# tomcreutz/slam-uwv_kalman_filters

Hardware: AMD Instinct MI355X
Metric: UKF predict+update steps/sec at batch=65536 PoseUKF instances, 1 & 8 GPU (higher is better)
Workload: dtype f64

## Files before the change

### slam-uwv_kalman_filters_amd/csrc/uwvk_psp_dev.hpp

```cpp
#pragma once
#include <cstddef>

#include "uwvk_pose_dev.hpp"
#include "uwvk_tiles.hpp"


#ifndef PSP_PAIR
#define PSP_PAIR 0
#endif
#ifndef PSP_NS
#define PSP_NS psp
#endif

namespace uwvk {
namespace PSP_NS {

constexpr int kLanes = PSP_PAIR ? 32 : 64;

UWVK_DEV void chain_prio_hi() { __builtin_amdgcn_s_setprio(1); }
UWVK_DEV void chain_prio_lo() { __builtin_amdgcn_s_setprio(0); }

template <int DOF>
struct PG {
  static constexpr int NP = DOF * (DOF + 1) / 2;
  static constexpr int NSLOT = (NP + kLanes - 1) / kLanes;
  static constexpr int N = 2 * DOF + 1;
  static constexpr int KP = 15;
  static constexpr int STG = 115;
};

template <int DOF>
struct alignas(16) PspSmem {
  double S[PG<DOF>::NP];
  double mu[Lay<DOF>::store];
  double stg[PG<DOF>::STG];
};
static_assert(sizeof(PspSmem<53>) <= 12800, "12 instances per CU");
static_assert(offsetof(PspSmem<53>, mu) == sizeof(double) * PG<53>::NP, "mu follows S");
static_assert(offsetof(PspSmem<53>, stg) == sizeof(double) * (PG<53>::NP + Lay<53>::store), "stg follows mu");
static_assert(offsetof(PspSmem<26>, mu) == sizeof(double) * PG<26>::NP, "mu follows S");
static_assert(offsetof(PspSmem<26>, stg) == sizeof(double) * (PG<26>::NP + Lay<26>::store), "stg follows mu");
constexpr int kPdLane0 = 27, kPdN = 27;
template <int DOF>
struct alignas(16) PspSmemPD : PspSmem<DOF> {
  double pS[32];
  double pm[32];
};
template <int DOF, int PD>
struct SmemT {
  using type = PspSmem<DOF>;
};
template <int DOF>
struct SmemT<DOF, 1> {
  using type = PspSmemPD<DOF>;
};
template <int DOF>
UWVK_DEV double* pd_ptr(PspSmem<DOF>&) {
  return nullptr;
}
template <int DOF>
UWVK_DEV double* pd_ptr(PspSmemPD<DOF>& s) {
  return s.pS;
}
UWVK_DEV constexpr int pd_dof(int d) { return d < 19 ? d : d + 27; }
UWVK_DEV constexpr int pd_store(int s) { return s < 20 ? s : s + 27; }

template <int DOF>
UWVK_DEV double* flat(PspSmem<DOF>& sm) {
  return reinterpret_cast<double*>(&sm);
}
template <int DOF>
UWVK_DEV const double* flat(const PspSmem<DOF>& sm) {
  return reinterpret_cast<const double*>(&sm);
}
template <int DOF>
constexpr int kFlatMu = PG<DOF>::NP;


UWVK_DEV int olane() {
  int l = PSP_PAIR ? ((int)threadIdx.x & 31) : (int)threadIdx.x;
  asm volatile("" : "+v"(l));
  return l;
}

template <class F>
UWVK_DEV constexpr unsigned long long lane_mask(F f) {
  unsigned long long m = 0;
  for (int i = 0; i < 64; i++)
    if (f(PSP_PAIR ? (i & 31) : i)) m |= 1ull << i;
  return m;
}
UWVK_DEV constexpr unsigned long long rep_mask(unsigned long long m) {
  return PSP_PAIR ? ((m & 0xFFFFFFFFull) | ((m & 0xFFFFFFFFull) << 32)) : m;
}
UWVK_DEV constexpr bool mask_needs_split(unsigned long long m) {
  return m >= 0xFFFFFFFF80000000ull && m < 0xFFFFFFFFFFFFFFF0ull;
}
UWVK_DEV bool lane_in_split(unsigned long long m) {
  unsigned lo = (unsigned)m, hi = (unsigned)(m >> 32);
  asm volatile("" : "+s"(lo), "+s"(hi));
  return __builtin_amdgcn_inverse_ballot_w64(((unsigned long long)hi << 32) | lo);
}
template <unsigned long long M>
UWVK_DEV bool lane_const() {
  if constexpr (mask_needs_split(M)) return lane_in_split(M);
  else return __builtin_amdgcn_inverse_ballot_w64(M);
}
#define LANE_IF(l, expr)                                                                                        \
  ({                                                                                                            \
    constexpr unsigned long long m_ = ::uwvk::PSP_NS::lane_mask([](int l) constexpr { return (bool)(expr); }); \
    ::uwvk::PSP_NS::lane_const<m_>();                                                                           \
  })
#define LANE_IN(m)                                                                     \
  (::uwvk::PSP_NS::mask_needs_split(::uwvk::PSP_NS::rep_mask(m))                       \
       ? ::uwvk::PSP_NS::lane_in_split(::uwvk::PSP_NS::rep_mask(m))                    \
       : __builtin_amdgcn_inverse_ballot_w64(::uwvk::PSP_NS::rep_mask(m)))
UWVK_DEV bool upper_half() { return lane_const<0xFFFFFFFF00000000ull>(); }
#if PSP_PAIR
template <int J>
UWVK_DEV double hbc(double v) {
  static_assert(J >= 0 && J < 16, "row_newbcast lane");
  int lo = __builtin_amdgcn_mov_dpp(__double2loint(v), 0x150 + J, 0xf, 0xf, false);
  int hi = __builtin_amdgcn_mov_dpp(__double2hiint(v), 0x150 + J, 0xf, 0xf, false);
  lo = __builtin_amdgcn_update_dpp(lo, lo, 0x142, 0xa, 0xf, false);
  hi = __builtin_amdgcn_update_dpp(hi, hi, 0x142, 0xa, 0xf, false);
  return __hiloint2double(hi, lo);
}
#endif
UWVK_DEV double hread(double v, int j) {
#if PSP_PAIR
  if (__builtin_constant_p(j) && j >= 0 && j < 16) {
    switch (j) {
      case 0: return hbc<0>(v);
      case 1: return hbc<1>(v);
      case 2: return hbc<2>(v);
      case 3: return hbc<3>(v);
      case 4: return hbc<4>(v);
      case 5: return hbc<5>(v);
      case 6: return hbc<6>(v);
      case 7: return hbc<7>(v);
      case 8: return hbc<8>(v);
      case 9: return hbc<9>(v);
      case 10: return hbc<10>(v);
      case 11: return hbc<11>(v);
      case 12: return hbc<12>(v);
      case 13: return hbc<13>(v);
      case 14: return hbc<14>(v);
      default: return hbc<15>(v);
    }
  }
  const double a = readlane_d(v, j), b = readlane_d(v, 32 + j);
  return upper_half() ? b : a;
#else
  return readlane_d(v, j);
#endif
}
UWVK_DEV int hlane(int j) { return PSP_PAIR ? j + ((int)threadIdx.x & 32) : j; }
UWVK_DEV constexpr int couple_c(int d) { return d < 3 ? d + 6 : (d >= 6 && d < 9 ? d + 3 : -1); }
template <int DOF>
UWVK_DEV constexpr unsigned long long col_ge_mask(int p, bool coupled) {
  unsigned long long m = 0;
  for (int l = 0; l < 64; l++) {
    const int jl = l < DOF ? l : DOF - 1, jc = couple_c(jl);
    const int j = coupled ? (jc >= 0 ? jc : jl) : jl;
    if (j >= p) m |= 1ull << l;
  }
  return m;
}
template <int DOF>
UWVK_DEV constexpr unsigned long long rows_store_mask(int p) {
  unsigned long long m = 0;
  for (int l = 0; l < 64; l++) {
    const int jl = l < DOF ? l : DOF - 1;
    if (!(couple_c(jl) >= 0) || l <= p) m |= 1ull << l;
  }
  return m;
}
template <class RL>
UWVK_DEV constexpr unsigned long long rows_mask() {
  unsigned long long m = 0;
  for (int k = 0; k < RL::NR; k++) m |= 1ull << RL::rows[k];
  return m;
}
template <class HM>
UWVK_DEV constexpr unsigned long long cols_mask() {
  unsigned long long m = 0;
  for (int k = 0; k < HM::NC; k++) m |= 1ull << HM::cols[k];
  for (int k = 1; k < HM::NC; k++)
    if (HM::cols[k] <= HM::cols[k - 1]) return 0;
  return m;
}
template <class RL>
UWVK_DEV constexpr bool rows_ascending() {
  for (int k = 1; k < RL::NR; k++)
    if (RL::rows[k] <= RL::rows[k - 1]) return false;
  return true;
}

template <int CTRL, int ROW, int BANK>
UWVK_DEV double dpp_d(double v) {
  const int lo = __builtin_amdgcn_update_dpp(0, __double2loint(v), CTRL, ROW, BANK, true);
  const int hi = __builtin_amdgcn_update_dpp(0, __double2hiint(v), CTRL, ROW, BANK, true);
  return __hiloint2double(hi, lo);
}
template <int NL = 64>
UWVK_DEV double wave_sum_dpp(double v) {
  double s = v + dpp_d<0x111, 0xf, 0xf>(v);
  s = s + dpp_d<0x112, 0xf, 0xf>(v);
  s = s + dpp_d<0x113, 0xf, 0xf>(v);
  s = s + dpp_d<0x114, 0xf, 0xe>(s);
  s = s + dpp_d<0x118, 0xf, 0xc>(s);
#if PSP_PAIR
  static_assert(NL <= 32, "pair: one instance per 32-lane half");
  if constexpr (NL <= 16) return hread(s, 15);
  s = s + dpp_d<0x142, 0xa, 0xf>(s);
  return hread(s, 31);
#else
  if constexpr (NL <= 16) return readlane_d(s, 15);
  s = s + dpp_d<0x142, 0xa, 0xf>(s);
  if constexpr (NL <= 32) return readlane_d(s, 31);
  s = s + dpp_d<0x143, 0xc, 0xf>(s);
  return readlane_d(s, 63);
#endif
}
UWVK_DEV double sk(double c) {
  asm volatile("" : "+s"(c));
  return c;
}
UWVK_DEV void so3_exp_psp(const double v[3], double o[4]) {
  const double t2 = v[0] * v[0] + v[1] * v[1] + v[2] * v[2];
  if (t2 < 0.0625) {
    const double u = 0.25 * t2;
    double s = u * sk(-1.0 / 39916800.0);
    s = s + sk(1.0 / 362880.0);
    s = fma(s, u, sk(-1.0 / 5040.0));
    s = fma(s, u, sk(1.0 / 120.0));
    s = fma(s, u, sk(-1.0 / 6.0));
    s = fma(s, u, 1.0);
    s = 0.5 * s;
    double c = u * sk(-1.0 / 3628800.0);
    c = c + sk(1.0 / 40320.0);
    c = fma(c, u, sk(-1.0 / 720.0));
    c = fma(c, u, sk(1.0 / 24.0));
    c = fma(c, u, -0.5);
    c = fma(c, u, 1.0);
    o[0] = c; o[1] = s * v[0]; o[2] = s * v[1]; o[3] = s * v[2];
  } else {
    so3_exp(v, o);
  }
}
UWVK_DEV void so3_log_psp(const double q[4], double o[3]) {
  double w = q[0], x = q[1], y = q[2], z = q[3];
  if (w < 0) { w = -w; x = -x; y = -y; z = -z; }
  const double n2 = x * x + y * y + z * z, w2 = w * w;
  if (n2 < 0.0025 * w2) {
    double iw = __builtin_amdgcn_rcp(w);
    iw = fma(iw, fma(-w, iw, 1.0), iw);
    iw = fma(iw, fma(-w, iw, 1.0), iw);
    const double r2 = n2 * (iw * iw);
    double a = r2 * sk(-1.0 / 13.0);
    a = fma(a, -r2, sk(1.0 / 11.0));
    a = fma(a, -r2, sk(1.0 / 9.0));
    a = fma(a, -r2, sk(1.0 / 7.0));
    a = fma(a, -r2, sk(1.0 / 5.0));
    a = fma(a, -r2, sk(1.0 / 3.0));
    a = fma(a, -r2, 1.0);
    const double k = 2.0 * a * iw;
    o[0] = k * x; o[1] = k * y; o[2] = k * z;
  } else {
    so3_log(q, o);
  }
}
template <int SR>
UWVK_DEV void qplus_psp(const double e[4], const double q[4], double o[4]) {
  if constexpr (SR) qmul(q, e, o);
  else qmul(e, q, o);
}
template <int SR>
UWVK_DEV void qboxminus_psp(const double a[4], const double b[4], double o[3]) {
  double bc[4] = {b[0], -b[1], -b[2], -b[3]}, r[4];
  if constexpr (SR) qmul(bc, a, r);
  else qmul(a, bc, r);
  so3_log_psp(r, o);
}

UWVK_DEV double swap_pair_d(double v) { return dpp_d<0xb1, 0xf, 0xf>(v); }

UWVK_DEV double sel3(double v0, double v1, double v2, int i) { return i == 0 ? v0 : (i == 1 ? v1 : v2); }
UWVK_DEV double sel6(double v0, double v1, double v2, double v3, double v4, double v5, int i) {
  return i < 3 ? sel3(v0, v1, v2, i) : sel3(v3, v4, v5, i - 3);
}

UWVK_DEV int pidx_sel(int p, int j, int Tj) { return j >= p ? Tj + p : p * (p + 1) / 2 + j; }
UWVK_DEV int pidx_sel_b(int p, int j, int Tj, bool ge) { return ge ? Tj + p : p * (p + 1) / 2 + j; }

UWVK_DEV void wsync() {
  __builtin_amdgcn_fence(__ATOMIC_RELEASE, "wavefront");
  __builtin_amdgcn_wave_barrier();
  __builtin_amdgcn_fence(__ATOMIC_ACQUIRE, "wavefront");
}

template <int R, int NL, int STRIDE>
UWVK_DEV void lds_sums(const double (&v)[R], double* buf, int l, double (&out)[R]) {
  static_assert(NL % 2 == 0 && R * NL <= 115, "transpose buffer (PG::STG)");
  const int c = l / STRIDE;
  if (l % STRIDE == 0 && c < NL) {
#pragma unroll
    for (int i = 0; i < R; i++) buf[i * NL + c] = v[i];
  }
  wsync();
  const double* row = buf + (l < R ? l : 0) * NL;
  double p[NL / 2];
#pragma unroll
  for (int k = 0; k < NL / 2; k++) p[k] = row[2 * k] + row[2 * k + 1];
#pragma unroll
  for (int w = 1; w < NL / 2; w *= 2)
#pragma unroll
    for (int k = 0; k + w < NL / 2; k += 2 * w) p[k] += p[k + w];
#pragma unroll
  for (int i = 0; i < R; i++) out[i] = hread(p[0], i);
}

#define PSP_PHASE(ph) \
  do {                \
    UWVK_STAMP(ph);   \
    l = olane();      \
  } while (0)

UWVK_DEV void psync() {
  __builtin_amdgcn_fence(__ATOMIC_RELEASE, "workgroup");
  __builtin_amdgcn_s_barrier();
  __builtin_amdgcn_fence(__ATOMIC_ACQUIRE, "workgroup");
}

UWVK_DEV constexpr bool scaled_dof(int d) { return d >= 12 && d != 18; }

template <int K, int J>
UWVK_DEV void pchol_step_lds(double (&a)[K], int r, bool& ok, double* col, double* rows, int q, double piv,
                             double inv_in, double& chk) {
  if constexpr (J < K) {
    ok = ok && (piv > 0.0);
    const double inv = rsqrt_f64(piv);
    a[J] = LANE_IF(r, r >= J) ? a[J] * inv : 0.0;
    double pnext = 0.0, invn = 0.0;
    if constexpr (J + 1 < K) {
      pnext = hread(a[J + 1] - a[J] * a[J], J + 1);
    }
    if constexpr (J + 1 < K) {
      constexpr int C0 = J + 1;
      double* const cj = col + (((C0 & 1) == 0) ? 1 : 0);
      static_assert(64 + 1 <= 115, "column slots (PG::STG)");
      cj[r & 63] = a[J];
      __builtin_amdgcn_fence(__ATOMIC_RELEASE, "wavefront");
      __builtin_amdgcn_wave_barrier();
      __builtin_amdgcn_fence(__ATOMIC_ACQUIRE, "wavefront");
#pragma unroll
      for (int c = C0; c < K; c++) a[c] -= a[J] * cj[c];
#pragma unroll
      for (int c = J + 1; c < K; c++) asm volatile("" : "+v"(a[c]));
    }
    pchol_step_lds<K, J + 1>(a, r, ok, col, rows, q, pnext, invn, chk);
  }
}

#if PSP_PAIR
template <int K, int J>
UWVK_DEV void pchol_step2_lds(double (&a)[K], const double (&f)[K], int r, bool& ok, double* col2, double piv) {
#pragma clang fp contract(off)
  if constexpr (J + 1 == K) {
    ok = ok && (piv > 0.0);
    const double inv = rsqrt_f64(piv);
    a[J] = LANE_IF(r, r >= J) ? a[J] * inv : 0.0;
  } else if constexpr (J + 1 < K) {
    static_assert(J + 1 < 16, "hbc lanes");
    ok = ok && (piv > 0.0);
    const double inv0 = rsqrt_f64(piv);
    a[J] = LANE_IF(r, r >= J) ? a[J] * inv0 : 0.0;
    a[J + 1] = fma(-a[J], hread(a[J], J + 1), a[J + 1]);
    const double piv1 = hread(a[J + 1], J + 1);
    ok = ok && (piv1 > 0.0);
    const double inv1 = rsqrt_f64(piv1);
    a[J + 1] = LANE_IF(r, r >= J + 1) ? a[J + 1] * inv1 : 0.0;
    double pnext = 0.0;
    if constexpr (J + 2 < K) {
      {
        const double t = J == 0 ? fma(f[J + 2], a[J + 2], -(a[J] * a[J])) : fma(-a[J], a[J], a[J + 2]);
        pnext = hread(fma(-a[J + 1], a[J + 1], t), J + 2);
      }
      static_assert(2 * kLanes + 1 <= 115, "column pair slots (PG::STG)");
      double* const c2 = static_cast<double*>(__builtin_assume_aligned(col2, 16));
      double* const w = static_cast<double*>(__builtin_assume_aligned(c2 + 2 * (r & (kLanes - 1)), 16));
      w[0] = a[J];
      w[1] = a[J + 1];
      __builtin_amdgcn_fence(__ATOMIC_RELEASE, "wavefront");
      __builtin_amdgcn_wave_barrier();
      __builtin_amdgcn_fence(__ATOMIC_ACQUIRE, "wavefront");
#pragma unroll
      for (int c = J + 2; c < K; c++) {
        const double t = J == 0 ? fma(f[c], a[c], -(a[J] * c2[2 * c])) : fma(-a[J], c2[2 * c], a[c]);
        a[c] = fma(-a[J + 1], c2[2 * c + 1], t);
      }
#pragma unroll
      for (int c = J + 2; c < K; c++) asm volatile("" : "+v"(a[c]));
    }
    pchol_step2_lds<K, J + 2>(a, f, r, ok, col2, pnext);
  }
}
#endif

constexpr int STG_ROWS = 0;

template <int DOF, int K, class RL>
UWVK_DEV bool pchol(const double* S, int r, double (&a)[K], double dl, double* stg) {
  const int rr = r < DOF ? r : DOF - 1;
  const double* Sr = S + rr * (rr + 1) / 2;
#if PSP_PAIR
  static_assert(K >= 2, "column pairs");
  double f[K];
#pragma unroll
  for (int c = 0; c < K; c++) {
    f[c] = scaled_dof(c) ? dl * hread(dl, c) : dl;
    a[c] = c < 2 ? Sr[c] * f[c] : Sr[c];
  }
#else
#pragma unroll
  for (int c = 0; c < K; c++) a[c] = Sr[c] * (scaled_dof(c) ? dl * hread(dl, c) : dl);
#endif
  bool ok = true;
  static_assert(rows_ascending<RL>(), "RL::rows ascending");
  constexpr unsigned long long rm = rep_mask(rows_mask<RL>());
  int q = (int)__builtin_amdgcn_mbcnt_hi((unsigned)(rm >> 32), __builtin_amdgcn_mbcnt_lo((unsigned)rm, 0u));
  if constexpr (PSP_PAIR) q -= upper_half() ? __builtin_popcount((unsigned)rm) : 0;
  static_assert(RL::NR >= 1 && STG_ROWS + RL::NR * K <= 115, "staging area (PG::STG)");
  const double p0 = hread(a[0], 0);
#if PSP_PAIR
  pchol_step2_lds<K, 0>(a, f, r, ok, stg + ((PG<DOF>::NP + Lay<DOF>::store) & 1), p0);
#else
  const double inv0 = rsqrt_f64(p0);
  double chk = fma(inv0, 0.0, 0.0);
  pchol_step_lds<K, 0>(a, r, ok, stg + STG_ROWS, stg + STG_ROWS, q, p0, inv0, chk);
#endif
  if (LANE_IN(rows_mask<RL>())) {
    double* rp = stg + STG_ROWS + q * K;
#pragma unroll
    for (int J = 0; J < K; J++) rp[J] = a[J];
  }
  psync();
  return ok;
}

template <int NR>
UWVK_DEV constexpr int row_pos(const int (&rows)[NR], int d) {
  for (int q = 0; q < NR; q++)
    if (rows[q] == d) return q;
  return -1;
}

template <class RL, int DOF, int K, int Q>
UWVK_DEV void gen_rows_q(const double* mu, const double* stg, int j, double sg, double (&v)[3], double* x) {
  if constexpr (Q < RL::NR) {
    constexpr int d = RL::rows[Q];
    const double l = stg[Q * K + j];
    if constexpr (d >= 3 && d < 6) {
      v[d - 3] = sg * l;
    } else {
      x[d2s(d)] = mu[d2s(d)] + sg * l;
    }
    gen_rows_q<RL, DOF, K, Q + 1>(mu, stg, j, sg, v, x);
  }
}
template <class RL>
UWVK_DEV constexpr bool has_rot() {
  for (int q = 0; q < RL::NR; q++)
    if (RL::rows[q] >= 3 && RL::rows[q] < 6) return true;
  return false;
}
template <class RL, int DOF, int K, int SR>
UWVK_DEV void gen_rows(const double* mu, const double* stg, int p, double x[Lay<DOF>::store]) {
  using L = Lay<DOF>;
#pragma unroll
  for (int s = 0; s < L::store; s++) x[s] = mu[s];
  if constexpr (K > 0) {
    const bool in = LANE_IF(p, p < 2 * K);
    const int j = in ? (p >> 1) : 0;
    const double sg = in ? (LANE_IF(p, (p & 1) != 0) ? -1.0 : 1.0) : 0.0;
    double v[3] = {0.0, 0.0, 0.0};
    gen_rows_q<RL, DOF, K, 0>(mu, stg, j, sg, v, x);
    if constexpr (has_rot<RL>()) {
      double e[4];
      so3_exp_psp(v, e);
      qplus_psp<SR>(e, mu + L::s_quat, x + L::s_quat);
    }
  }
}

template <int DOF, int SR>
UWVK_DEV void proc_orientation(const double x[Lay<DOF>::store], const PoseShared& sh, const ProcCtx& c, double o[4]) {
  using L = Lay<DOF>;
  const double dl = x[L::s_pos] * sh.inv_rm;
  double sl, cl;
  if (fabs(dl) < 0.01) {
    const double u = dl * dl;
    double sd = fma(fma(fma(u * sk(1.0 / 362880.0) + sk(-1.0 / 5040.0), u, sk(1.0 / 120.0)), u, sk(-1.0 / 6.0)), u, 1.0) * dl;
    double cd = fma(fma(fma(u * sk(1.0 / 40320.0) + sk(-1.0 / 720.0), u, sk(1.0 / 24.0)), u, -0.5), u, 1.0);
    sl = sh.slat0 * cd + sh.clat0 * sd;
    cl = sh.clat0 * cd - sh.slat0 * sd;
  } else {
    sincos(sh.lat0 + dl, &sl, &cl);
  }
  const double er[3] = {kEarthW * cl, 0.0, kEarthW * sl};
  double wb[3], wn[3];
#pragma unroll
  for (int i = 0; i < 3; i++) wb[i] = c.w[i] - x[L::s_bg + i];
  qrot(x + L::s_quat, wb, wn);
#pragma unroll
  for (int i = 0; i < 3; i++) wn[i] = (wn[i] - er[i]) * c.dt;
  double e[4];
  so3_exp_psp(wn, e);
  qplus_psp<SR>(e, x + L::s_quat, o);
}

UWVK_DEV double proc_vect_lane(int s, const double* mu, const ProcCtx& c) {
  const double x = mu[s];
  const double y = mu[c.vpart >= 0 ? c.vpart : s];
  const double d = c.vpart >= 0 ? y : c.nt_lane * (x - c.off_lane);
  return (c.vpart >= 0 || c.nt_lane != 0.0) ? x + c.dt * d : x;
}

template <int DOF>
UWVK_DEV double tan_ntau_sel(int d, const PoseShared& sh) {
  using L = Lay<DOF>;
  double nt = 0.0;
  nt = (d >= L::d_bg && d < L::d_bg + 3) ? sh.ntau[0] : nt;
  nt = (d >= L::d_ba && d < L::d_ba + 3) ? sh.ntau[1] : nt;
  if constexpr (L::has_params) {
    nt = (d >= L::d_inertia && d < L::d_inertia + 9) ? sh.ntau[2] : nt;
    nt = (d >= L::d_lin && d < L::d_lin + 9) ? sh.ntau[3] : nt;
    nt = (d >= L::d_quad && d < L::d_quad + 9) ? sh.ntau[4] : nt;
  }
  nt = (d >= L::d_wv && d < L::d_wv + 4) ? sh.ntau[5] : nt;
  nt = (d >= L::d_badcp && d < L::d_badcp + 2) ? sh.ntau[6] : nt;
  nt = (d == L::d_rho) ? sh.ntau[7] : nt;
  return nt;
}
UWVK_DEV constexpr int proc_couple(int d) { return d < 3 ? d + 6 : (d >= 6 && d < 9 ? d + 3 : -1); }

struct PredRows {
  static constexpr int NR = 7;
  static constexpr int rows[NR] = {0, 3, 4, 5, 12, 13, 14};
};

struct LaneQ {
  double q0, q1, q2;
};
template <int DOF, int PD = 0>
UWVK_DEV LaneQ lane_q(const double* fq, int l) {
  const double2* f2 = reinterpret_cast<const double2*>(fq);
  LaneQ q{0.0, 0.0, 0.0};
  if (l < DOF) {
    q.q0 = f2[pidx(l, l)].y;
    if (l >= 1) q.q1 = f2[pidx(l, l - 1)].y;
    if (l >= 2) q.q2 = f2[pidx(l, l - 2)].y;
  }
  if constexpr (PD && !PSP_PAIR) {
    if (l >= kPdLane0 && l < kPdLane0 + kPdN) q.q0 = f2[PG<DOF>::NP + (l - kPdLane0)].y;
  }
  return q;
}

template <int DOF, int QM = 0, int SR = 0, int PD = 0>
UWVK_DEV bool psp_predict(PspSmem<DOF>& sm, const PoseShared& sh, const ProcCtx& pc, const double* Q,
                          const double* fq, double& ds, double& ids, const LaneQ& lq,
                          Stamper* st = nullptr, double* px = nullptr) {
  using L = Lay<DOF>;
  using G = PG<DOF>;
  constexpr int K = G::KP;
  static_assert(!PD || (DOF == 26 && QM == 1), "PD: the 26-DOF layout, lane-resident Q");
  constexpr int NW = PD ? 53 : DOF;
  int l = olane();
  const double dt = pc.dt, dt2 = dt * dt;
  double qo_lane = 0.0;
  if (LANE_IF(l, l < 9)) {
    double R[9];
    qmatrix(sm.mu + L::s_quat, R);
    const int r = l / 3, c = l % 3;
    double Rr[3], Rc[3];
#pragma unroll
    for (int m = 0; m < 3; m++) {
      Rr[m] = sel3(R[m], R[3 + m], R[6 + m], r);
      Rc[m] = sel3(R[m], R[3 + m], R[6 + m], c);
    }
    double s = 0.0;
#pragma unroll
    for (int k = 0; k < 3; k++) {
      double u = 0.0;
#pragma unroll
      for (int m = 0; m < 3; m++) u += Rr[m] * sh.q_ori[m * 3 + k];
      s += u * Rc[k];
    }
    qo_lane = s;
  }
  const double vs0 = sm.mu[L::s_vel], vs1 = sm.mu[L::s_vel + 1], vs2 = 10 * sm.mu[L::s_vel + 2];
  const double wv_add = sh.p.water_velocity_scale * (vs0 * vs0 + vs1 * vs1 + vs2 * vs2) * dt;
  double a[K];
  chain_prio_hi();
  const bool ok = pchol<DOF, K, PredRows>(sm.S, l, a, ds, sm.stg);
  chain_prio_lo();
  PSP_PHASE(20);
  const bool pt = LANE_IF(l, l < 2 * K), ctr = LANE_IF(l, l == 2 * K);
  double o[4];
  {
    double x[L::store];
    gen_rows<PredRows, DOF, K, SR>(sm.mu, sm.stg + STG_ROWS, l, x);
    proc_orientation<DOF, SR>(x, sh, pc, o);
  }
  PSP_PHASE(21);
  constexpr double wc = 1.0 + 2.0 * (NW - K);
  double mq[4];
#pragma unroll
  for (int i = 0; i < 4; i++) mq[i] = hread(o[i], 2 * K);
  {
    int it = 0;
    double nrm;
// ... 1241 lines not shown
```

### slam-uwv_kalman_filters_amd/csrc/uwvk_psp_pair.hip

```cpp
#define PSP_PAIR 1
#define PSP_NS psp2
#ifndef PSP_PAIR_WAVES
#define PSP_PAIR_WAVES 3
#endif
#include <algorithm>
#include <atomic>

#define UWVK_POSE_KERNEL_BODIES
#include "uwvk_pose_kernels.hpp"
#include "uwvk_psp_dev.hpp"
#include "uwvk_psp.hpp"

namespace uwvk {
namespace psp2 {

UWVK_DEV int half() { return (int)(threadIdx.x >> 5) & 1; }

struct PUnit {
  int64_t unit, e0, e1, tslot;
  int chunk;
};
UWVK_DEV PUnit ticket_unit(const EpochArgs& ea, uint32_t u) {
  PUnit t{(int64_t)u, ea.first, ea.first + ea.count, 0, -1};
  if (ea.chunks > 1 && (int64_t)u >= ea.tail0) {
    const uint32_t q = u - (uint32_t)ea.tail0, m = (uint32_t)ea.r_x;
    const uint32_t k = q / m, r = q - k * m;
    t.unit = ea.tail0 + r;
    t.chunk = (int)k;
    t.tslot = r;
    t.e0 = ea.first + ea.count * k / ea.chunks;
    t.e1 = ea.first + ea.count * (k + 1) / ea.chunks;
  }
  return t;
}
UWVK_DEV uint32_t ticket_issue(const EpochArgs& ea) {
  uint32_t v = 0;
  if (lane_id() == 0) v = __hip_atomic_fetch_add(ea.ticket, 1u, __ATOMIC_RELAXED, __HIP_MEMORY_SCOPE_AGENT);
  return v;
}
UWVK_DEV uint32_t ticket_value(const EpochArgs& ea, uint32_t v) {
  return __builtin_amdgcn_readfirstlane(v) - ea.ticket_base;
}
UWVK_DEV bool tail_wait(uint32_t* f, uint32_t want, uint32_t bound) {
  uint32_t n = 0;
  if (lane_id() == 0) {
    while (__hip_atomic_load(f, __ATOMIC_RELAXED, __HIP_MEMORY_SCOPE_AGENT) != want && ++n < bound)
      __builtin_amdgcn_s_sleep(64);
  }
  n = __builtin_amdgcn_readfirstlane(n);
  __builtin_amdgcn_wave_barrier();
  __builtin_amdgcn_fence(__ATOMIC_ACQUIRE, "agent");
  return n < bound;
}
UWVK_DEV void tail_signal(const EpochArgs& ea, int64_t t, int chunk) {
  __builtin_amdgcn_fence(__ATOMIC_RELEASE, "agent");
  __builtin_amdgcn_wave_barrier();
  if (lane_id() == 0)
    __hip_atomic_store(ea.tail_flag + t, ea.tag * 16u + (uint32_t)(chunk + 1), __ATOMIC_RELAXED,
                       __HIP_MEMORY_SCOPE_AGENT);
}

UWVK_DEV int pd_pidx(int e) {
  int i = (int)((sqrtf(8.0f * (float)e + 1.0f) - 1.0f) * 0.5f);
  if (((i + 1) * (i + 2)) / 2 <= e) i++;
  if ((i * (i + 1)) / 2 > e) i--;
  const int j = e - (i * (i + 1)) / 2;
  const int I = pd_dof(i), J = pd_dof(j);
  return (I * (I + 1)) / 2 + J;
}
UWVK_DEV constexpr int pd_diag53(int t) { return ((19 + t) * (20 + t)) / 2 + 19 + t; }
constexpr int kPdTab = PG<26>::NSLOT * kLanes;
static_assert(PG<53>::NP <= 65536, "16-bit table entries");
UWVK_DEV void pd_tab_fill(unsigned short* tab, int l) {
#pragma unroll
  for (int t = 0; t < PG<26>::NSLOT; t++) {
    const int e = l + kLanes * t;
    tab[e] = (unsigned short)(e < PG<26>::NP ? pd_pidx(e) : 0);
  }
  psync();
}

UWVK_DEV void lane_proc(const PoseBufs& b, const PoseShared& sh, int64_t inst, int s, ProcCtx& pc) {
  using L = Lay<26>;
  const uwvk_pose_parameter& P = sh.p;
  pc.vpart = s < 3 ? L::s_vel + s : ((s >= L::s_vel && s < L::s_vel + 3) ? L::s_acc + s - L::s_vel : -1);
  pc.nt_lane = 0.0;
  pc.off_lane = 0.0;
  int k = -1;
  if (s >= L::s_bg && s < L::s_bg + 3) { pc.nt_lane = sh.ntau[0]; pc.off_lane = P.gyro_bias_offset[s - L::s_bg]; }
  if (s >= L::s_ba && s < L::s_ba + 3) { pc.nt_lane = sh.ntau[1]; pc.off_lane = P.acc_bias_offset[s - L::s_ba]; }
  if (s >= L::s_wv && s < L::s_wv + 4) pc.nt_lane = sh.ntau[5];
  if (s >= L::s_badcp && s < L::s_badcp + 2) pc.nt_lane = sh.ntau[6];
  if (s == L::s_rho) { k = 27; pc.nt_lane = sh.ntau[7]; }
  if (k >= 0) pc.off_lane = b.off[inst * 28 + k];
  pc.nt_tan = 0.0;
  if (s < 26 && scaled_dof(s)) pc.nt_tan = tan_ntau_sel<26>(s, sh);
}

struct ParLane {
  double q;
  double off;
  double nt;
};
UWVK_DEV ParLane par_lane(const PoseBufs& b, const PoseShared& sh, int64_t inst, int t) {
  ParLane p{0.0, 0.0, 0.0};
  if (t < kPdN) {
    p.q = reinterpret_cast<const double2*>(b.Qp)[PG<26>::NP + t].y;
    p.off = b.off[inst * 28 + t];
    p.nt = t < 9 ? sh.ntau[2] : (t < 18 ? sh.ntau[3] : sh.ntau[4]);
  }
  return p;
}
UWVK_DEV void par_epoch(double* px, int t, double dt, const ParLane& p) {
  if (t < kPdN) {
    const double a = 1.0 + dt * p.nt;
    const double v = px[t], m = px[32 + t];
    px[t] = a * (a * v) + p.q;
    px[32 + t] = m + dt * (p.nt * (m - p.off));
  }
}

UWVK_DEV void load_pair(PspSmem<26>& sm, double* px, const unsigned short* tab, const PoseBufs& b, int64_t inst,
                        int l) {
  using G = PG<26>;
  const double* gs = b.sigma + inst * (int64_t)PG<53>::NP;
  const double* gm = b.mu + inst * (int64_t)Lay<53>::store;
  double v[G::NSLOT];
#pragma unroll
  for (int t = 0; t < G::NSLOT; t++) {
    const int e = l + kLanes * t;
    v[t] = e < G::NP ? gs[tab[e]] : 0.0;
  }
  const double m = l < Lay<26>::store ? gm[pd_store(l)] : 0.0;
  const bool pl = l < kPdN;
  const double ps = pl ? gs[pd_diag53(l)] : 0.0, pm = pl ? gm[20 + l] : 0.0;
#pragma unroll
  for (int t = 0; t < G::NSLOT; t++) {
    const int e = l + kLanes * t;
    if (e < G::NP) sm.S[e] = v[t];
  }
  if (l < Lay<26>::store) sm.mu[l] = m;
  if (pl) {
    px[l] = ps;
    px[32 + l] = pm;
  }
  psync();
}
UWVK_DEV void store_pair(const PspSmem<26>& sm, const double* px, const unsigned short* tab, const PoseBufs& b,
                         int64_t inst, int l) {
  using G = PG<26>;
  double* gs = b.sigma + inst * (int64_t)PG<53>::NP;
  double* gm = b.mu + inst * (int64_t)Lay<53>::store;
  static_assert(G::NSLOT * kLanes <= G::NP + Lay<26>::store + PG<26>::STG, "slot over-read stays in PspSmem");
  double v[G::NSLOT];
#pragma unroll
  for (int t = 0; t < G::NSLOT; t++) v[t] = flat(sm)[l + kLanes * t];
  const double m = flat(sm)[kFlatMu<26> + l];
  const bool pl = l < kPdN;
  const double ps = px[l], pm = px[32 + l];
#pragma unroll
  for (int t = 0; t < G::NSLOT; t++) {
    const int e = l + kLanes * t;
    if (e < G::NP) gs[tab[e]] = v[t];
  }
  if (l < Lay<26>::store) gm[pd_store(l)] = m;
  if (pl) {
    gs[pd_diag53(l)] = ps;
    gm[20 + l] = pm;
  }
}

UWVK_DEV void load_pair26(PspSmem<26>& sm, const PoseBufs& b, int64_t inst, int l) {
  using G = PG<26>;
  const double* gs = b.sigma + inst * (int64_t)G::NP;
  const double* gm = b.mu + inst * (int64_t)Lay<26>::store;
  double v[G::NSLOT];
#pragma unroll
  for (int t = 0; t < G::NSLOT; t++) {
    const int e = l + kLanes * t;
    v[t] = e < G::NP ? gs[e] : 0.0;
  }
  const double m = l < Lay<26>::store ? gm[l] : 0.0;
#pragma unroll
  for (int t = 0; t < G::NSLOT; t++) {
    const int e = l + kLanes * t;
    if (e < G::NP) sm.S[e] = v[t];
  }
  if (l < Lay<26>::store) sm.mu[l] = m;
  psync();
}
UWVK_DEV void store_pair26(const PspSmem<26>& sm, const PoseBufs& b, int64_t inst, int l) {
  using G = PG<26>;
  double* gs = b.sigma + inst * (int64_t)G::NP;
  double* gm = b.mu + inst * (int64_t)Lay<26>::store;
  double v[G::NSLOT];
#pragma unroll
  for (int t = 0; t < G::NSLOT; t++) v[t] = flat(sm)[l + kLanes * t];
  const double m = flat(sm)[kFlatMu<26> + l];
#pragma unroll
  for (int t = 0; t < G::NSLOT; t++) {
    const int e = l + kLanes * t;
    if (e < G::NP) gs[e] = v[t];
  }
  if (l < Lay<26>::store) gm[l] = m;
}

template <int M>
UWVK_DEV void copy_zr(const double* zin, const double* Rin, double (&z)[M], double (&R)[M * M]) {
#pragma unroll
  for (int k = 0; k < M; k++) z[k] = zin[k];
#pragma unroll
  for (int k = 0; k < M * M; k++) R[k] = Rin[k];
}
UWVK_DEV bool finite_n(const double* a, int n) {
  bool ok = true;
  for (int i = 0; i < n; i++) ok = ok && __builtin_isfinite(a[i]);
  return ok;
}
UWVK_DEV const PoseShared& shared_for_epoch(const PoseBufs& b) {
  using CP = const __attribute__((address_space(4))) PoseShared*;
  CP p = (CP)b.shared;
  asm volatile("" : "+s"(p));
  return *(const PoseShared*)p;
}

template <int SR, int EVS, int PD>
__global__ __launch_bounds__(64) __attribute__((amdgpu_waves_per_eu(PSP_PAIR_WAVES, PSP_PAIR_WAVES)))
void k_psp_epoch_pair(PoseBufs b, PoseShared sh0, EpochArgs ea) {
  __shared__ PspSmemPD<26> smx[2];
  __shared__ unsigned short pdx[PD ? kPdTab : 1];
  const int h = half();
  PspSmem<26>& sm = smx[h];
  double* const px = smx[h].pS;
  constexpr int NW = PD ? 53 : 26;
  const int64_t B = b.batch;
  const uint32_t grid = gridDim.x;
  uint32_t u = blockIdx.x;
  if constexpr (PD) pd_tab_fill(pdx, olane());
#pragma unroll 1
  while (u < ea.units) {
    const PUnit tu = ticket_unit(ea, u);
    if (tu.chunk > 0 && !tail_wait(ea.tail_flag + tu.tslot, ea.tag * 16u + (uint32_t)tu.chunk, ea.wait_bound)) {
      if ((threadIdx.x & 31) == 0) {
        __hip_atomic_fetch_or(b.status + 2 * tu.unit + h, UWVK_ST_SCHEDULE, __ATOMIC_RELAXED, __HIP_MEMORY_SCOPE_AGENT);
        __hip_atomic_store(ea.fault, 1u, __ATOMIC_RELAXED, __HIP_MEMORY_SCOPE_SYSTEM);
      }
      u = grid + ticket_value(ea, ticket_issue(ea));
      psync();
      continue;
    }
    const int l = olane();
    const int64_t inst = 2 * tu.unit + h;
    const int64_t e_begin = tu.e0, e_end = tu.e1;
    bool ok = true, nan = false;
    uint32_t cnt[4] = {0, 0, 0, 0};
    ProcCtx pc;
    for (int k = 0; k < 3; k++) pc.w[k] = b.rot[inst * 3 + k];
    {
      double dtv = ea.dt;
      asm volatile("" : "+v"(dtv));
      pc.dt = dtv;
    }
    pc.off = nullptr;
    lane_proc(b, *b.shared, inst, l, pc);
    const ParLane pl = PD ? par_lane(b, *b.shared, inst, l) : ParLane{0.0, 0.0, 0.0};
    const LaneQ lq = lane_q<26, 0>(b.Qp, l);
    uint32_t fl_n = 0;
    double g_n[3] = {0, 0, 0}, a_n[3] = {0, 0, 0};
    auto fetch = [&](int64_t e) {
      fl_n = ea.flags[e];
#pragma unroll
      for (int k = 0; k < 3; k++) {
        g_n[k] = ea.gyro[(e * B + inst) * 3 + k];
        a_n[k] = ea.acc[(e * B + inst) * 3 + k];
      }
    };
    if (e_end > e_begin) fetch(e_begin);
    if constexpr (PD) load_pair(sm, px, pdx, b, inst, l);
    else load_pair26(sm, b, inst, l);
    double ds = 1.0, ids = 1.0;
    if (tu.chunk > 0) {
      const double2 c = reinterpret_cast<const double2*>(ea.tail_carry)[tu.tslot * 64 + lane_id()];
      ds = c.x;
      ids = c.y;
    }
    uint32_t vn = ticket_issue(ea);
#pragma unroll 1
    for (int64_t e = e_begin; e < e_end; e++) {
      const uint32_t fl = fl_n;
      const double g[3] = {g_n[0], g_n[1], g_n[2]}, za[3] = {a_n[0], a_n[1], a_n[2]};
      if (e + 1 < e_end) fetch(e + 1);
      if (finite_n(g, 3)) {
        for (int k = 0; k < 3; k++) pc.w[k] = g[k];
      } else {
        nan = true;
      }
      const PoseShared& sh = shared_for_epoch(b);
      if (((e - ea.first) & 1023) == 1023) psp_fold<26, 0>(sm, ds, ids);
      bool sok = psp_predict<26, 1, SR, PD>(sm, sh, pc, b.Q, b.Qp, ds, ids, lq, nullptr, px);
      if constexpr (PD) par_epoch(px, l, pc.dt, pl);
      ok = ok && sok;
      if (fl & UWVK_EV_ACC) {
        if (finite_n(za, 3)) {
          double z[3], R[9];
          copy_zr<3>(za, sh.log_acc_cov, z, R);
          psp_update<26, SR, PAcc<26>, NW>(sm, z, R, 0, PAcc<26>{}, &sok, ds, ids);
          ok = ok && sok;
        } else {
          nan = true;
        }
      }
      if (fl & UWVK_EV_DVL) {
        const double* zp = ea.dvl + ((int64_t)ea.dvl_index[e] * B + inst) * 3;
        if (finite_n(zp, 3)) {
          double z[3], R[9];
          copy_zr<3>(zp, sh.log_dvl_cov, z, R);
          cnt[0] += psp_update<26, SR, PVel<26>, NW>(sm, z, R, 0, PVel<26>{}, &sok, ds, ids);
          ok = ok && sok;
        } else {
          nan = true;
        }
      }
      if constexpr (EVS == 0) {
        if (fl & UWVK_EV_ADCP) {
          for (int c = 0; c < ea.cells; c++) {
            const double* zp = ea.adcp + (((int64_t)ea.a_index[e] * ea.cells + c) * B + inst) * 2;
            if (!finite_n(zp, 2)) {
              nan = true;
              continue;
            }
            double z[2] = {zp[0], zp[1]}, R[4] = {ea.adcp_cov[0], ea.adcp_cov[1], ea.adcp_cov[2], ea.adcp_cov[3]};
            PWater<26> hw;
            hw.cw = ea.cw[c];
            cnt[2] += psp_update<26, SR, PWater<26>, NW>(sm, z, R, 1, hw, &sok, ds, ids);
            ok = ok && sok;
          }
        }
      }
    }
    if (l == 0) {
      const uint32_t bits = (ok ? 0u : UWVK_ST_NOTPD) | (nan ? UWVK_ST_NAN : 0u);
      if (bits) __hip_atomic_fetch_or(b.status + inst, bits, __ATOMIC_RELAXED, __HIP_MEMORY_SCOPE_AGENT);
      if (e_end > e_begin) {
        b.rot[inst * 3] = pc.w[0]; b.rot[inst * 3 + 1] = pc.w[1]; b.rot[inst * 3 + 2] = pc.w[2];
      }
      if (ea.accept_counts)
        for (int k = 0; k < 4; k++) ea.accept_counts[inst * 4 + k] += cnt[k];
    }
    const uint32_t un = grid + ticket_value(ea, vn);
    const PUnit tn = ticket_unit(ea, u);
    const bool hand = tn.chunk >= 0 && tn.chunk + 1 < ea.chunks;
    if (hand) {
      double* c = ea.tail_carry + (tn.tslot * 64 + lane_id()) * 2;
      c[0] = ds;
      c[1] = ids;
      psync();
    } else {
      psp_fold<26, 0>(sm, ds, ids);
    }
    if constexpr (PD) store_pair(sm, px, pdx, b, inst, l);
    else store_pair26(sm, b, inst, l);
    if (hand) tail_signal(ea, tn.tslot, tn.chunk);
    u = un;
    psync();
  }
}

}

template <int SR, int PD>
static hipError_t launch_pair_sr(hipStream_t st, const PoseBufs& b, const PoseShared& sh, const EpochArgs& ea,
                                 int64_t grid, uint32_t ev_any) {
  const dim3 g((unsigned)grid), t(64);
  if (ev_any & UWVK_EV_PRESSURE) return hipErrorInvalidValue;
  if (ev_any & UWVK_EV_ADCP) hipLaunchKernelGGL((psp2::k_psp_epoch_pair<SR, 0, PD>), g, t, 0, st, b, sh, ea);
  else hipLaunchKernelGGL((psp2::k_psp_epoch_pair<SR, 1, PD>), g, t, 0, st, b, sh, ea);
  return hipGetLastError();
}

hipError_t launch_psp_epoch_pair(hipStream_t st, const PoseBufs& b, const PoseShared& sh, const EpochArgs& ea,
                                 int64_t grid, uint32_t ev_any, int pd) {
  if (!sh.q_simple || !ea.ticket || grid <= 0) return hipErrorInvalidValue;
  if (pd) return sh.so3_right ? launch_pair_sr<1, 1>(st, b, sh, ea, grid, ev_any)
                              : launch_pair_sr<0, 1>(st, b, sh, ea, grid, ev_any);
  return sh.so3_right ? launch_pair_sr<1, 0>(st, b, sh, ea, grid, ev_any)
                      : launch_pair_sr<0, 0>(st, b, sh, ea, grid, ev_any);
}

int64_t psp_pair_slots(int device) {
  int per_cu = 0, cus = 0;
  if (hipOccupancyMaxActiveBlocksPerMultiprocessor(&per_cu, (const void*)psp2::k_psp_epoch_pair<1, 1, 1>, 64, 0) !=
          hipSuccess ||
      hipDeviceGetAttribute(&cus, hipDeviceAttributeMultiprocessorCount, device) != hipSuccess)
    return 0;
  return (int64_t)per_cu * cus;
}

}
```

Baseline: 434.2 million.

## Hoist per-unit lane setup, simplify pair broadcasts and unpredicate slot loads

Several micro-optimizations to the paired-wave PoseUKF kernel. The per-lane constant setup (lane_proc, par_lane, lane_q) moves out of the unit loop, and only the per-instance offsets are reloaded for each unit. In lds_sums for the pair variant, each 16-lane row computes its own sum, so the broadcast needs one DPP move instead of two. Load and store loops drop their bounds predicates for full slots and clamp indices instead of branching. Together these trim instructions and register pressure per unit and per update, at the cost of extra live registers held across the loop.

New measurement: 433.1 million (median of 2 runs). No clear change (-0.3%).

```diff
diff --git a/slam-uwv_kalman_filters_amd/csrc/uwvk_psp_dev.hpp b/slam-uwv_kalman_filters_amd/csrc/uwvk_psp_dev.hpp
--- a/slam-uwv_kalman_filters_amd/csrc/uwvk_psp_dev.hpp
+++ b/slam-uwv_kalman_filters_amd/csrc/uwvk_psp_dev.hpp
@@ -124,6 +124,13 @@
   int hi = __builtin_amdgcn_mov_dpp(__double2hiint(v), 0x150 + J, 0xf, 0xf, false);
   lo = __builtin_amdgcn_update_dpp(lo, lo, 0x142, 0xa, 0xf, false);
   hi = __builtin_amdgcn_update_dpp(hi, hi, 0x142, 0xa, 0xf, false);
+  return __hiloint2double(hi, lo);
+}
+template <int J>
+UWVK_DEV double hbc1(double v) {
+  static_assert(J >= 0 && J < 16, "row_newbcast lane");
+  const int lo = __builtin_amdgcn_mov_dpp(__double2loint(v), 0x150 + J, 0xf, 0xf, false);
+  const int hi = __builtin_amdgcn_mov_dpp(__double2hiint(v), 0x150 + J, 0xf, 0xf, false);
   return __hiloint2double(hi, lo);
 }
 #endif
@@ -300,6 +307,15 @@
   __builtin_amdgcn_fence(__ATOMIC_ACQUIRE, "wavefront");
 }
 
+#if PSP_PAIR
+template <int R, int I = 0>
+UWVK_DEV void row_reads(double p, double (&out)[R]) {
+  if constexpr (I < R) {
+    out[I] = hbc1<I>(p);
+    row_reads<R, I + 1>(p, out);
+  }
+}
+#endif
 template <int R, int NL, int STRIDE>
 UWVK_DEV void lds_sums(const double (&v)[R], double* buf, int l, double (&out)[R]) {
   static_assert(NL % 2 == 0 && R * NL <= 115, "transpose buffer (PG::STG)");
@@ -309,7 +325,13 @@
     for (int i = 0; i < R; i++) buf[i * NL + c] = v[i];
   }
   wsync();
-  const double* row = buf + (l < R ? l : 0) * NL;
+#if PSP_PAIR
+  static_assert(R <= 16, "one adding lane per row of 16");
+  const int la = l & 15;
+#else
+  const int la = l;
+#endif
+  const double* row = buf + (la < R ? la : 0) * NL;
   double p[NL / 2];
 #pragma unroll
   for (int k = 0; k < NL / 2; k++) p[k] = row[2 * k] + row[2 * k + 1];
@@ -317,8 +339,12 @@
   for (int w = 1; w < NL / 2; w *= 2)
 #pragma unroll
     for (int k = 0; k + w < NL / 2; k += 2 * w) p[k] += p[k + w];
+#if PSP_PAIR
+  row_reads<R>(p[0], out);
+#else
 #pragma unroll
   for (int i = 0; i < R; i++) out[i] = hread(p[0], i);
+#endif
 }
 
 #define PSP_PHASE(ph) \
diff --git a/slam-uwv_kalman_filters_amd/csrc/uwvk_psp_pair.hip b/slam-uwv_kalman_filters_amd/csrc/uwvk_psp_pair.hip
--- a/slam-uwv_kalman_filters_amd/csrc/uwvk_psp_pair.hip
+++ b/slam-uwv_kalman_filters_amd/csrc/uwvk_psp_pair.hip
@@ -80,19 +80,17 @@
   psync();
 }
 
-UWVK_DEV void lane_proc(const PoseBufs& b, const PoseShared& sh, int64_t inst, int s, ProcCtx& pc) {
+UWVK_DEV void lane_proc(const PoseShared& sh, int s, ProcCtx& pc) {
   using L = Lay<26>;
   const uwvk_pose_parameter& P = sh.p;
   pc.vpart = s < 3 ? L::s_vel + s : ((s >= L::s_vel && s < L::s_vel + 3) ? L::s_acc + s - L::s_vel : -1);
   pc.nt_lane = 0.0;
   pc.off_lane = 0.0;
-  int k = -1;
   if (s >= L::s_bg && s < L::s_bg + 3) { pc.nt_lane = sh.ntau[0]; pc.off_lane = P.gyro_bias_offset[s - L::s_bg]; }
   if (s >= L::s_ba && s < L::s_ba + 3) { pc.nt_lane = sh.ntau[1]; pc.off_lane = P.acc_bias_offset[s - L::s_ba]; }
   if (s >= L::s_wv && s < L::s_wv + 4) pc.nt_lane = sh.ntau[5];
   if (s >= L::s_badcp && s < L::s_badcp + 2) pc.nt_lane = sh.ntau[6];
-  if (s == L::s_rho) { k = 27; pc.nt_lane = sh.ntau[7]; }
-  if (k >= 0) pc.off_lane = b.off[inst * 28 + k];
+  if (s == L::s_rho) pc.nt_lane = sh.ntau[7];
   pc.nt_tan = 0.0;
   if (s < 26 && scaled_dof(s)) pc.nt_tan = tan_ntau_sel<26>(s, sh);
 }
@@ -102,14 +100,20 @@
   double off;
   double nt;
 };
-UWVK_DEV ParLane par_lane(const PoseBufs& b, const PoseShared& sh, int64_t inst, int t) {
+UWVK_DEV ParLane par_lane(const PoseBufs& b, const PoseShared& sh, int t) {
   ParLane p{0.0, 0.0, 0.0};
   if (t < kPdN) {
     p.q = reinterpret_cast<const double2*>(b.Qp)[PG<26>::NP + t].y;
-    p.off = b.off[inst * 28 + t];
     p.nt = t < 9 ? sh.ntau[2] : (t < 18 ? sh.ntau[3] : sh.ntau[4]);
   }
   return p;
+}
+struct UnitOff {
+  double par, rho;
+};
+UWVK_DEV UnitOff unit_offsets(const PoseBufs& b, int64_t inst, int l) {
+  const double* o = b.off + inst * 28;
+  return UnitOff{o[l < kPdN ? l : 27], o[27]};
 }
 UWVK_DEV void par_epoch(double* px, int t, double dt, const ParLane& p) {
   if (t < kPdN) {
@@ -120,24 +124,23 @@
   }
 }
 
+UWVK_DEV constexpr bool slot_full(int t) { return kLanes * (t + 1) <= PG<26>::NP; }
 UWVK_DEV void load_pair(PspSmem<26>& sm, double* px, const unsigned short* tab, const PoseBufs& b, int64_t inst,
                         int l) {
   using G = PG<26>;
   const double* gs = b.sigma + inst * (int64_t)PG<53>::NP;
   const double* gm = b.mu + inst * (int64_t)Lay<53>::store;
   double v[G::NSLOT];
+  const bool pl = l < kPdN;
+  static_assert(G::NSLOT * kLanes <= kPdTab, "every slot has a table entry");
+#pragma unroll
+  for (int t = 0; t < G::NSLOT; t++) v[t] = gs[tab[l + kLanes * t]];
+  const double m = gm[pd_store(l < Lay<26>::store ? l : 0)];
+  const double ps = gs[pd_diag53(pl ? l : 0)], pm = gm[20 + (pl ? l : 0)];
 #pragma unroll
   for (int t = 0; t < G::NSLOT; t++) {
     const int e = l + kLanes * t;
-    v[t] = e < G::NP ? gs[tab[e]] : 0.0;
-  }
-  const double m = l < Lay<26>::store ? gm[pd_store(l)] : 0.0;
-  const bool pl = l < kPdN;
-  const double ps = pl ? gs[pd_diag53(l)] : 0.0, pm = pl ? gm[20 + l] : 0.0;
-#pragma unroll
-  for (int t = 0; t < G::NSLOT; t++) {
-    const int e = l + kLanes * t;
-    if (e < G::NP) sm.S[e] = v[t];
+    if (slot_full(t) || e < G::NP) sm.S[e] = v[t];
   }
   if (l < Lay<26>::store) sm.mu[l] = m;
   if (pl) {
@@ -161,7 +164,7 @@
 #pragma unroll
   for (int t = 0; t < G::NSLOT; t++) {
     const int e = l + kLanes * t;
-    if (e < G::NP) gs[tab[e]] = v[t];
+    if (slot_full(t) || e < G::NP) gs[tab[e]] = v[t];
   }
   if (l < Lay<26>::store) gm[pd_store(l)] = m;
   if (pl) {
@@ -178,13 +181,13 @@
 #pragma unroll
   for (int t = 0; t < G::NSLOT; t++) {
     const int e = l + kLanes * t;
-    v[t] = e < G::NP ? gs[e] : 0.0;
-  }
-  const double m = l < Lay<26>::store ? gm[l] : 0.0;
+    v[t] = gs[slot_full(t) || e < G::NP ? e : 0];
+  }
+  const double m = gm[l < Lay<26>::store ? l : 0];
 #pragma unroll
   for (int t = 0; t < G::NSLOT; t++) {
     const int e = l + kLanes * t;
-    if (e < G::NP) sm.S[e] = v[t];
+    if (slot_full(t) || e < G::NP) sm.S[e] = v[t];
   }
   if (l < Lay<26>::store) sm.mu[l] = m;
   psync();
@@ -200,7 +203,7 @@
 #pragma unroll
   for (int t = 0; t < G::NSLOT; t++) {
     const int e = l + kLanes * t;
-    if (e < G::NP) gs[e] = v[t];
+    if (slot_full(t) || e < G::NP) gs[e] = v[t];
   }
   if (l < Lay<26>::store) gm[l] = m;
 }
@@ -237,6 +240,20 @@
   const uint32_t grid = gridDim.x;
   uint32_t u = blockIdx.x;
   if constexpr (PD) pd_tab_fill(pdx, olane());
+  ProcCtx pc0;
+  ParLane pl0{0.0, 0.0, 0.0};
+  LaneQ lq;
+  {
+    const int l0 = olane();
+    pc0.w[0] = pc0.w[1] = pc0.w[2] = 0.0;
+    double dtv = ea.dt;
+    asm volatile("" : "+v"(dtv));
+    pc0.dt = dtv;
+    pc0.off = nullptr;
+    lane_proc(*b.shared, l0, pc0);
+    if constexpr (PD) pl0 = par_lane(b, *b.shared, l0);
+    lq = lane_q<26, 0>(b.Qp, l0);
+  }
 #pragma unroll 1
   while (u < ea.units) {
     const PUnit tu = ticket_unit(ea, u);
@@ -254,17 +271,11 @@
     const int64_t e_begin = tu.e0, e_end = tu.e1;
     bool ok = true, nan = false;
     uint32_t cnt[4] = {0, 0, 0, 0};
-    ProcCtx pc;
+    const UnitOff uo = unit_offsets(b, inst, l);
+    ProcCtx pc = pc0;
     for (int k = 0; k < 3; k++) pc.w[k] = b.rot[inst * 3 + k];
-    {
-      double dtv = ea.dt;
-      asm volatile("" : "+v"(dtv));
-      pc.dt = dtv;
-    }
-    pc.off = nullptr;
-    lane_proc(b, *b.shared, inst, l, pc);
-    const ParLane pl = PD ? par_lane(b, *b.shared, inst, l) : ParLane{0.0, 0.0, 0.0};
-    const LaneQ lq = lane_q<26, 0>(b.Qp, l);
+    pc.off_lane = LANE_IF(l, l == Lay<26>::s_rho) ? uo.rho : pc0.off_lane;
+    const ParLane pl{pl0.q, uo.par, pl0.nt};
     uint32_t fl_n = 0;
     double g_n[3] = {0, 0, 0}, a_n[3] = {0, 0, 0};
     auto fetch = [&](int64_t e) {
@@ -298,7 +309,7 @@
       const PoseShared& sh = shared_for_epoch(b);
       if (((e - ea.first) & 1023) == 1023) psp_fold<26, 0>(sm, ds, ids);
       bool sok = psp_predict<26, 1, SR, PD>(sm, sh, pc, b.Q, b.Qp, ds, ids, lq, nullptr, px);
-      if constexpr (PD) par_epoch(px, l, pc.dt, pl);
+      if constexpr (PD) par_epoch(px, olane(), pc.dt, pl);
       ok = ok && sok;
       if (fl & UWVK_EV_ACC) {
         if (finite_n(za, 3)) {
```
